# wthanone/kmerLSH

Hardware: AMD Instinct MI355X
Metric: k-mers·iterations/sec (LSH+cluster loop), 10M k-mers × 64 samples (higher is better)
Workload: dtype f32

## Files before the change

kmerlsh_amd/csrc/klsh_engine.cpp:

```cpp
#include <hip/hip_runtime.h>
#include <stdint.h>
#include <stdio.h>
#include <stdlib.h>
#include <stddef.h>
#include <string.h>

#include <algorithm>
#include <array>
#include <atomic>
#include <cstring>
#include <chrono>
#include <cmath>
#include <deque>
#include <functional>
#include <numeric>
#include <string>
#include <thread>
#include <vector>

#include "klsh.h"
#include "klsh_comm.h"
#include "klsh_internal.h"

extern "C" {
// ... 1668 lines not shown
  KLSH_HIP(hipSetDevice(ctx->device));
  std::string err;
  klsh::Comm* c = klsh::make_rccl_comm(rank, world, id, ctx->device, &err);
  if (!c) return fail(KLSH_E_HIP, err);
  c->timeout_s = ctx->comm_timeout_s;
  ctx->release_shard();
  delete ctx->comm;
  ctx->comm = c;
  return 0;
}

int klsh_comm_init_local(klsh_ctx** ctxs, int world) {
  if (!ctxs || world < 1 || world > klsh::kMaxRanks) return fail(KLSH_E_ARG, "bad argument");
  for (int r = 0; r < world; ++r)
    if (!ctxs[r]) return fail(KLSH_E_ARG, "null context");
  std::vector<klsh::Comm*> cs(world);
  klsh::make_local_comms(world, cs.data());
  for (int r = 0; r < world; ++r) {
    ctxs[r]->release_shard();
    delete ctxs[r]->comm;
    ctxs[r]->comm = cs[r];
  }
  return 0;
}

int klsh_set_option(klsh_ctx* ctx, const char* name, int64_t value) {
  if (!ctx || !name) return fail(KLSH_E_ARG, "null argument");
  const std::string n(name);
  auto flag = [&](bool* f) {
    *f = value != 0;
    return 0;
  };
  auto grid = [&](uint32_t* g) {
    if (value < 0 || value > (1 << 20)) return fail(KLSH_E_ARG, n + " must be in [0, 2^20]");
    *g = (uint32_t)value;
    return 0;
  };
  if (n == "shard_min_rows") {
    if (value < 0) return fail(KLSH_E_ARG, "shard_min_rows must be >= 0");
    ctx->shard_min_rows = (uint64_t)value;
    return 0;
  }
  if (n == "phase_timing") return flag(&ctx->phase_timing);
  if (n == "kernel_timing") return flag(&ctx->kernel_timing);
  if (n == "tail_batch") return flag(&ctx->tail_batch);
  if (n == "huge_fold") return flag(&ctx->huge_fold_always);
  if (n == "tail_local") return flag(&ctx->tail_local);
  if (n == "hyperplane_async") {
    if (value != 0 && value != 1) return fail(KLSH_E_ARG, "hyperplane_async must be 0 or 1");
    ctx->hyperplane_async = (uint32_t)value;
    return 0;
  }
  if (n == "hyperplane_window") {
    if (value < 0) return fail(KLSH_E_ARG, "hyperplane_window must be >= 0");
    ctx->hyperplane_window = (uint64_t)value;
    return 0;
  }
  if (n == "progress") {
    if (value < 0 || value > INT32_MAX) return fail(KLSH_E_ARG, "progress must be >= 0");
    ctx->progress = (int)value;
    return 0;
  }
  if (n == "stop_after") {
    if (value < 0 || value > INT32_MAX) return fail(KLSH_E_ARG, "stop_after must be in [0, 2^31)");
    ctx->stop_after = (int)value;
    return 0;
  }
  if (n == "projection") {
    if (value != klsh::kProjAuto && value != klsh::kProjPacked)
      return fail(KLSH_E_ARG, "projection must be 0 (default) or 1 (exact packed chains)");
    KLSH_HIP(hipSetDevice(ctx->device));
    ctx->pw.variant = (uint32_t)value;
    return ctx->apply_projection_variant();
  }
  if (n == "wide_gram") {
    if (value != 0 && value != 8 && value != 16 && value != 32 && value != 64)
      return fail(KLSH_E_ARG, "wide_gram must be 0, 8, 16, 32 or 64");
    ctx->mw.wide_gram = (uint32_t)value;
    return 0;
  }
  if (n == "wide_unrolled") {
    if (value != 0 && value != 1) return fail(KLSH_E_ARG, "wide_unrolled must be 0 or 1");
    ctx->pw.wide_rolled = value ? 0u : 1u;
    return 0;
  }
  if (n == "long_runs") {
    if (value != 0 && value != 1 && value != 4) return fail(KLSH_E_ARG, "long_runs must be 0, 1 or 4");
    ctx->mw.long_off = value == 1 ? 0u : value == 0 ? 1u : 4u;
    KLSH_HIP(hipSetDevice(ctx->device));
    return ctx->cap_slots ? ctx->ensure_long(ctx->cap_slots, ctx->d) : 0;
  }
  if (n == "comm_timeout_s") {
    if (value <= 0) return fail(KLSH_E_ARG, "comm_timeout_s must be > 0");
    ctx->comm_timeout_s = (double)value;
    if (ctx->comm) ctx->comm->timeout_s = (double)value;
    return 0;
  }
  if (n == "kmc_chunk_records") {
    if (value < 0) return fail(KLSH_E_ARG, "kmc_chunk_records must be >= 0");
    ctx->kmc.chunk_records = (uint64_t)value;
    return 0;
  }
  if (n == "kmc_ordinal_base") {
    if (value < 0 || value > (1ll << 48)) return fail(KLSH_E_ARG, "kmc_ordinal_base must be in [0, 2^48]");
    ctx->kmc.ordinal_base = (uint64_t)value;
    return 0;
  }
  if (n == "kmc_keep_first") {
    if (!value) std::vector<uint64_t>().swap(ctx->kmc.first);
    return flag(&ctx->kmc.keep_first);
  }
  if (n == "kcount_batch_reads") {
    if (value < 0) return fail(KLSH_E_ARG, "kcount_batch_reads must be >= 0");
    ctx->kcount.batch_reads = (uint64_t)value;
    return 0;
  }
  if (n == "kcount_table_slots") {
    if (value != 0 && (value < 1024 || value > (1ll << 32) || (value & (value - 1))))
      return fail(KLSH_E_ARG, "kcount_table_slots must be 0 or a power of two in [1024, 2^32]");
    ctx->kcount.table_slots = (uint64_t)value;
    return 0;
  }
  if (n == "kcount_db_prefix") {
    if (value < -1 || value > 15) return fail(KLSH_E_ARG, "kcount_db_prefix must be in [-1, 15]");
    ctx->kcount.db_prefix = (int)value;
    return 0;
  }
  if (n == "kcount_db_chunk_records") {
    if (value < 0) return fail(KLSH_E_ARG, "kcount_db_chunk_records must be >= 0");
    ctx->kcount.db_chunk_records = (uint64_t)value;
    return 0;
  }
  if (n == "kcount_keep_listing") {
    if (!value) {
      std::vector<std::vector<uint64_t>>().swap(ctx->kcount.values);
      std::vector<std::vector<uint32_t>>().swap(ctx->kcount.counts);
    }
    return flag(&ctx->kcount.keep_listing);
  }
  if (n == "h16_grid") return grid(&ctx->pw.h16_grid);
  if (n == "h16_segcap") return grid(&ctx->pw.segcap);
  if (n == "wide_grid") return grid(&ctx->pw.wide_grid);
  if (n == "fix_grid") return grid(&ctx->pw.fix_grid);
  if (n == "small_grid") return grid(&ctx->mw.small_grid);
  if (n == "tail_big_groups") return grid(&ctx->mw.tail_nbig);
  if (n == "tail_small_groups") return grid(&ctx->mw.tail_nsmall);
  if (n == "wide_group_grid") return grid(&ctx->mw.wide_group_grid);
  if (n == "small_screen_grid") return grid(&ctx->mw.screen_grid);
  if (n == "grid_cap") {
    if (int e = grid(&ctx->mw.grid_cap)) return e;
    ctx->kmc.grid_cap = ctx->kcount.grid_cap = ctx->mw.grid_cap;
    return 0;
  }
  if (n == "tail_merge_rows") {
    if (value < 0 || value > (1 << 22)) return fail(KLSH_E_ARG, "tail_merge_rows must be in [0, 2^22]");
    ctx->mw.tail_max = (uint32_t)value;
    return 0;
  }
  if (n == "tail_screen") {
    if (value != 0 && value != 1) return fail(KLSH_E_ARG, "tail_screen must be 0 or 1");
    ctx->mw.tail_screen = (uint32_t)value;
    return 0;
  }
  if (n == "tail_screen_grid") return grid(&ctx->mw.tail_screen_grid);
  if (n == "tail_big_screen") {
    if (value != 0 && value != 1) return fail(KLSH_E_ARG, "tail_big_screen must be 0 or 1");
    ctx->mw.tail_big_screen = (uint32_t)value;
    return 0;
  }
  if (n == "hip_events") {
    if (value != 0 && value != 1) return fail(KLSH_E_ARG, "hip_events must be 0 or 1");
    ctx->hip_events = value != 0;
    return 0;
  }
  if (n == "small_screen") {
    if (value != 0 && value != 1) return fail(KLSH_E_ARG, "small_screen must be 0 or 1");
    ctx->mw.small_screen = (uint32_t)value;
    return 0;
  }
  return fail(KLSH_E_ARG, "unknown option " + n);
}

int klsh_get_option(klsh_ctx* ctx, const char* name, int64_t* value) {
  if (!ctx || !name || !value) return fail(KLSH_E_ARG, "null argument");
  const std::string n(name);
  if (n == "shard_min_rows") *value = (int64_t)ctx->shard_min_rows;
  else if (n == "phase_timing") *value = ctx->phase_timing;
  else if (n == "kernel_timing") *value = ctx->kernel_timing;
  else if (n == "tail_batch") *value = ctx->tail_batch;
  else if (n == "huge_fold") *value = ctx->huge_fold_always;
  else if (n == "tail_local") *value = ctx->tail_local;
  else if (n == "hyperplane_window") *value = (int64_t)ctx->hyperplane_window;
  else if (n == "hyperplane_async") *value = ctx->hyperplane_async;
  else if (n == "stop_after") *value = ctx->stop_after;
  else if (n == "progress") *value = ctx->progress;
  else if (n == "projection") *value = ctx->pw.variant;
  else if (n == "comm_timeout_s") *value = (int64_t)ctx->comm_timeout_s;
  else if (n == "kmc_chunk_records") *value = (int64_t)ctx->kmc.chunk_records;
  else if (n == "kmc_ordinal_base") *value = (int64_t)ctx->kmc.ordinal_base;
  else if (n == "kmc_keep_first") *value = ctx->kmc.keep_first;
  else if (n == "kmc_decode_launches") *value = (int64_t)ctx->kmc.decode_launches;
  else if (n == "kmc_high_sort") *value = ctx->kmc.high_sort;
  else if (n == "kcount_batch_reads") *value = (int64_t)ctx->kcount.batch_reads;
  else if (n == "kcount_table_slots") *value = (int64_t)ctx->kcount.table_slots;
  else if (n == "kcount_keep_listing") *value = ctx->kcount.keep_listing;
  else if (n == "kcount_batches") *value = (int64_t)ctx->kcount.batches;
  else if (n == "kcount_rehashes") *value = (int64_t)ctx->kcount.rehashes;
  else if (n == "kcount_peak_slots") *value = (int64_t)ctx->kcount.peak_slots;
  else if (n == "kcount_window") *value = (int64_t)klsh::kKcountWindow;
  else if (n == "kcount_db_prefix") *value = ctx->kcount.db_prefix;
  else if (n == "kcount_db_chunk_records") *value = (int64_t)ctx->kcount.db_chunk_records;
  else if (n == "kcount_db_chunks") *value = (int64_t)ctx->kcount.db_chunks;
  else if (n == "kcount_db_prefix_used") *value = ctx->kcount.db_prefix_used;
  else if (n == "h16_grid") *value = ctx->pw.h16_grid;
  else if (n == "h16_segcap") *value = ctx->pw.segcap;
  else if (n == "wide_grid") *value = ctx->pw.wide_grid;
  else if (n == "fix_grid") *value = ctx->pw.fix_grid;
  else if (n == "small_grid") *value = ctx->mw.small_grid;
  else if (n == "tail_big_groups") *value = ctx->mw.tail_nbig;
  else if (n == "tail_small_groups") *value = ctx->mw.tail_nsmall;
  else if (n == "wide_group_grid") *value = ctx->mw.wide_group_grid;
  else if (n == "small_screen_grid") *value = ctx->mw.screen_grid;
  else if (n == "grid_cap") *value = ctx->mw.grid_cap;
  else if (n == "tail_merge_rows") *value = klsh::tail_merge_max(ctx->mw);
  else if (n == "small_screen") *value = ctx->mw.small_screen;
  else if (n == "hip_events") *value = ctx->hip_events ? 1 : 0;
  else if (n == "tail_screen") *value = ctx->mw.tail_screen;
  else if (n == "tail_screen_grid") *value = ctx->mw.tail_screen_grid;
  else if (n == "tail_big_screen") *value = ctx->mw.tail_big_screen;
  else if (n == "long_runs") *value = ctx->mw.long_off == 1u ? 0 : ctx->mw.long_off == 0u ? 1 : ctx->mw.long_off;
  else if (n == "wide_gram") *value = ctx->mw.wide_gram;
  else if (n == "wide_unrolled") *value = ctx->pw.wide_rolled ? 0 : 1;
  else if (n == "fp16_image") *value = ctx->rows.xh != nullptr;
  else if (n == "last_hash_kernel") *value = ctx->last_hash_kernel;
  else if (n == "last_hash_close_pairs") *value = (int64_t)ctx->last_hash_close;
  else return fail(KLSH_E_ARG, "unknown option " + n);
  return 0;
}

int klsh_comm_info(klsh_ctx* ctx, int* rank, int* world) {
  if (!ctx) return fail(KLSH_E_ARG, "null ctx");
  if (rank) *rank = ctx->rank();
  if (world) *world = ctx->world();
  return 0;
}

int klsh_count(klsh_ctx* ctx, uint64_t* n_rows, uint64_t* n_members) {
  if (!ctx) return fail(KLSH_E_ARG, "null ctx");
  if (!ctx->loaded) return fail(KLSH_E_STATE, "nothing loaded");
  if (n_rows) *n_rows = ctx->n_live;
  if (n_members) {
    KLSH_HIP(hipSetDevice(ctx->device));
    std::vector<uint32_t> ord(ctx->n_live), cnt(ctx->slots);
    if (ctx->n_live)
      KLSH_HIP(hipMemcpy(ord.data(), ctx->order, 4 * ctx->n_live, hipMemcpyDeviceToHost));
    if (ctx->slots)
      KLSH_HIP(hipMemcpy(cnt.data(), ctx->rows.cnt, 4 * ctx->slots, hipMemcpyDeviceToHost));
    uint64_t m = 0;
    for (uint32_t sl : ord) m += cnt[sl];
    *n_members = m;
  }
  return 0;
}

int klsh_result(klsh_ctx* ctx, float* rows, uint64_t* member_offsets, uint64_t* member_ids) {
  if (!ctx) return fail(KLSH_E_ARG, "null ctx");
  if (!ctx->loaded) return fail(KLSH_E_STATE, "nothing loaded");
  KLSH_HIP(hipSetDevice(ctx->device));
  const uint64_t n = ctx->n_live;
  hipStream_t s = ctx->stream;
  if (rows && n) {
    float* tmp = nullptr;
    if (int e = dalloc(&tmp, n * (uint64_t)ctx->d)) return e;
    klsh::launch_gather_rows(ctx->rows, ctx->order, (uint32_t)n, tmp, s);
    hipError_t e1 = hipMemcpyAsync(rows, tmp, sizeof(float) * n * ctx->d, hipMemcpyDeviceToHost, s);
    hipError_t e2 = hipStreamSynchronize(s);
    dfree(tmp);
    if (e1 != hipSuccess || e2 != hipSuccess) return fail(KLSH_E_HIP, "result rows copy");
  }
  if (member_offsets || member_ids) {
    std::vector<uint32_t> ord(n), head(ctx->slots), nxt(ctx->members);
    if (n) KLSH_HIP(hipMemcpy(ord.data(), ctx->order, 4 * n, hipMemcpyDeviceToHost));
    if (ctx->slots)
      KLSH_HIP(hipMemcpy(head.data(), ctx->rows.head, 4 * ctx->slots, hipMemcpyDeviceToHost));
    if (ctx->members)
      KLSH_HIP(hipMemcpy(nxt.data(), ctx->rows.nxt, 4 * ctx->members, hipMemcpyDeviceToHost));
    uint64_t m = 0;
    for (uint64_t i = 0; i < n; ++i) {
      if (member_offsets) member_offsets[i] = m;
      if (ord[i] >= ctx->slots) return fail(KLSH_E_STATE, "corrupt live order");
      for (uint32_t node = head[ord[i]]; node != klsh::kNil; node = nxt[node]) {
        if (node >= ctx->members || m >= ctx->members)
          return fail(KLSH_E_STATE, "corrupt member list");
        if (member_ids) member_ids[m] = ctx->ids[node];
        ++m;
      }
    }
    if (member_offsets) member_offsets[n] = m;
  }
  return 0;
}

int klsh_row_state(klsh_ctx* ctx, float* nrm, uint32_t* cnt, uint16_t* image,
                   uint64_t* pad_nonzero, uint64_t* bad_links) {
  if (!ctx) return fail(KLSH_E_ARG, "null ctx");
  if (!ctx->loaded) return fail(KLSH_E_STATE, "nothing loaded");
  KLSH_HIP(hipSetDevice(ctx->device));
  KLSH_HIP(hipStreamSynchronize(ctx->stream));
  const uint64_t n = ctx->n_live, S = ctx->slots, M = ctx->members;
  const int d = ctx->d, dp = ctx->dp;
  std::vector<uint32_t> ord(n);
  if (n) KLSH_HIP(hipMemcpy(ord.data(), ctx->order, 4 * n, hipMemcpyDeviceToHost));
  for (uint32_t sl : ord)
    if (sl >= S) return fail(KLSH_E_STATE, "corrupt live order");
  if (nrm && n) {
// ... 289 lines not shown
```

kmerlsh_amd/csrc/klsh_internal.h:

```cpp
#pragma once

#include <hip/hip_ext.h>
#include <hip/hip_runtime_api.h>
#include <stdint.h>
#include <stdio.h>

#include <vector>

#include "klsh.h"

namespace klsh {

constexpr uint32_t kInvalid = 0xFFFFFFFFu;
constexpr uint32_t kNil = 0xFFFFFFFFu;
constexpr int kMaxHyperplanes = 32;
constexpr int kScanTile = 4096;
uint64_t sort_ws_words(uint64_t slots);
constexpr uint32_t kScanStatusWord = 64;
constexpr uint64_t kScanSumsWord = kScanStatusWord + 2ull * (1ull << 20);
inline uint64_t scan_ws_words(uint64_t slots) {
  return kScanSumsWord + (256 * slots) / kScanTile + 1024;
}

constexpr int kBigClasses = 4;
// ... 54 lines not shown
  KStampBlock* blk;
  int set;
  int fold;
  int phase = -1;
};
constexpr KTime kNoTime{nullptr, 0, -1, -1};

struct MergeWork {
  uint2* cls[kGroupClasses];
  uint2* act[kGroupClasses];
  uint32_t screened;
  uint2* big[kBigClasses];
  uint2* huge;
  uint2* over;
  uint32_t* tile_sums;
  RunCounters* rc;
  uint32_t* run_ws;
  uint32_t* dlist;
  uint32_t* mark;
  uint32_t stamp;
  uint32_t big896_aux;
  uint32_t huge_cap;
  uint32_t huge_fold;
  uint64_t* long_P;
  uint32_t long_groups;
  uint32_t long_off = 4;
  uint32_t small_grid;
  uint32_t tail_nbig;
  uint32_t tail_nsmall;
  uint32_t wide_group_grid;
  uint32_t screen_grid;
  uint32_t wide_gram = 32;
  uint32_t small_screen = 1;
  uint32_t tail_screen = 1;
  uint32_t tail_big_screen = 1;
  uint32_t big_screen = 0;
  float bs_s_star = 0.0f, bs_m0 = 0.0f, bs_a2 = 0.0f;
  uint32_t tail_screen_grid;
  uint32_t tail_max;
  uint32_t grid_cap = 0;
  hipStream_t aux[3];
  KTime kt;
  hipEvent_t small_ev[2];
  hipEvent_t fork;
  hipEvent_t join[3];
};
constexpr int kMergeStreams = 3;
inline uint32_t cap_grid(uint32_t g, uint32_t cap) { return cap && g > cap ? cap : g; }
constexpr uint32_t kLongRows = 4096;
inline bool long_ok(int d) { return d == 16 || d == 32; }
inline uint32_t tail_merge_max(const MergeWork& w) { return w.tail_max ? w.tail_max : (1u << 22); }

struct Rows {
  float* x;
  float* nrm;
  uint32_t* cnt;
  uint32_t* head;
  uint32_t* tail;
  uint32_t* nxt;
  int d;
  int dp;
  uint16_t* xh = nullptr;
};
inline bool shadow_width_ok(int d) { return d == 16 || d == 32 || d == 64; }

struct Decider {
  float s_star, s_lo, s_hi;
  uint32_t fast;
  float g_lo, g_hi;
};
constexpr float kGramMargin = 1.0e-4f;
Decider make_decider(float thr);

struct ProjectWork {
  uint2* fix;
  uint32_t* ws;
  uint32_t cap;
  uint32_t h16_grid;
  uint32_t wide_grid;
  uint32_t fix_grid;
  uint32_t segcap;
  uint32_t variant;
  uint32_t wide_rolled;
};
constexpr uint32_t kProjAuto = 0, kProjPacked = 1, kProjScreen = 2;
constexpr uint32_t kH16Grid = 2048;

bool project_device_n_ok(int d);
void launch_project_device_n(const Rows& r, const uint32_t* slots, uint32_t* keys, uint32_t n_max,
                             const float* W, const uint32_t* n_dev, hipStream_t s,
                             KTime kt = kNoTime, const uint32_t* woff_dev = nullptr,
                             const ProjectWork* pw = nullptr);

enum ProjKernel : int { kPkNone = -1, kPkPacked = 0, kPkH16 = 1, kPkWide = 2 };
int launch_project(const Rows& r, const uint32_t* slots, uint32_t* keys, uint32_t n,
                   const float* W, int h, uint32_t key_or, hipStream_t s,
                   const ProjectWork* pw = nullptr, KTime kt = kNoTime);

void radix_sort(uint32_t* k0, uint32_t* v0, uint32_t* k1, uint32_t* v1, uint32_t n, int bits,
                uint32_t* ws, uint32_t** out_k, uint32_t** out_v, hipStream_t s,
                KTime kt = kNoTime, const uint32_t* n_dev = nullptr);

void launch_merge(const Rows& r, const uint32_t* key, uint32_t* slots, uint32_t lo, uint32_t hi,
                  float thr, int bucket_thr, const MergeWork& w, Counters* ctr, hipStream_t s,
                  const uint32_t* n_dev = nullptr, bool runs_ready = false);

const uint32_t* radix_sort_top(const uint32_t* k0, const uint32_t* v0, uint32_t* k1, uint32_t* v1,
                               uint32_t n, int bits, uint32_t* ws, hipStream_t s, KTime kt,
                               const uint32_t* n_dev);
void launch_tail_local(const uint32_t* kin, const uint32_t* vin, uint32_t* kout, uint32_t* vout,
                       const uint32_t* dtot, int bits, int bucket_thr, const MergeWork& w,
                       hipStream_t s);
constexpr int kTailTopBits = 9;
constexpr int kTailLowBits = 19 - kTailTopBits > 10 ? 19 - kTailTopBits : 10;
inline bool tail_local_ok(uint32_t n_max, int bits) {
  return n_max <= (1u << 20) && bits > kTailTopBits && bits <= kTailTopBits + kTailLowBits;
}

constexpr int kRunListCount = kGroupClasses + kBigClasses + 2;
void launch_runs(const uint32_t* key, uint32_t lo, uint32_t n, int bucket_thr, const MergeWork& w,
                 hipStream_t s, const uint32_t* n_dev = nullptr);

struct Publish {
  Counters* host;
  uint32_t* seq_host;
  uint32_t seq;
  uint32_t* n_next;
  uint32_t* woff = nullptr;
};

struct LookBack {
  unsigned long long* status;
  mutable uint32_t epoch;
};

void launch_compact(const uint32_t* slots, uint32_t n, uint32_t* out, uint32_t* tile_sums,
                    Counters* ctr, hipStream_t s, const Publish* pub = nullptr,
                    RunCounters* rc = nullptr, KTime kt = kNoTime,
                    const LookBack* lb = nullptr, const uint32_t* n_dev = nullptr);
void launch_stamp_fold(KStampBlock* blk, int set, hipStream_t s);
void launch_publish_words(const uint32_t* a, uint32_t na, const uint32_t* b, uint32_t nb,
                          uint32_t* dst, uint32_t* seq_host, uint32_t seq, hipStream_t s);

void launch_convert(const Rows& r, const uint16_t* counts, uint32_t bs, const float* lut,
                    const float* v_kmers, uint32_t* keep, uint32_t* order, uint32_t* tile_sums,
                    Counters* ctr, hipStream_t s);

void launch_norms(const Rows& r, uint32_t n, hipStream_t s);
void launch_shadow_build(const Rows& r, uint64_t n, hipStream_t s);


void launch_gather_rows(const Rows& r, const uint32_t* order, uint32_t n, float* out,
                        hipStream_t s);

void launch_fp_selftest(const float* a, const float* b, uint32_t n, float* sqrt_out,
                        float* div_out, hipStream_t s);

constexpr int kMaxBinBits = 12;
constexpr int kMaxRanks = 64;

void launch_bin_hist(const uint32_t* keys, uint32_t n, int shift, uint32_t nbins, uint32_t* hist,
                     hipStream_t s, uint32_t grid_cap = 0);
void launch_bin_split(const uint32_t* hist_all, int world, uint32_t nbins, uint64_t total,
                      uint32_t* owner, uint32_t* cntmat, hipStream_t s);
int launch_partition(const uint32_t* keys, const uint32_t* slots, uint32_t n, int shift,
                     const uint32_t* owner, int world, uint32_t* counts, uint32_t* tile_sums,
// ... 115 lines not shown
```

kmerlsh_amd/csrc/klsh_kernels.hip:

```cpp
#include <hip/hip_runtime.h>

#include <stdlib.h>

#include <string>
#include <type_traits>

#include "klsh_device.h"

namespace klsh {

typedef float f32x2 __attribute__((ext_vector_type(2)));


__device__ __forceinline__ void pk_mac_lo(f32x2& acc, f32x2 w, f32x2 x) {
  f32x2 t;
  asm("v_pk_mul_f32 %1, %2, %3 op_sel_hi:[1,0]\n\tv_pk_add_f32 %0, %0, %1"
      : "+v"(acc), "=&v"(t) : "v"(w), "v"(x));
}
__device__ __forceinline__ void pk_mac_hi(f32x2& acc, f32x2 w, f32x2 x) {
  f32x2 t;
  asm("v_pk_mul_f32 %1, %2, %3 op_sel:[0,1] op_sel_hi:[1,1]\n\tv_pk_add_f32 %0, %0, %1"
      : "+v"(acc), "=&v"(t) : "v"(w), "v"(x));
}

// ... 144 lines not shown
  const int d4 = d & ~3;
  for (int k = 0; k < d4; k += 4) {
    f32x2 x01[RPL], x23[RPL];
#pragma unroll
    for (int r = 0; r < RPL; ++r) {
      const float4 v = *reinterpret_cast<const float4*>(x[r] + k);
      x01[r] = (f32x2){v.x, v.y};
      x23[r] = (f32x2){v.z, v.w};
    }
    column(swq + (size_t)k * nq, x01, false);
    column(swq + (size_t)(k + 1) * nq, x01, true);
    column(swq + (size_t)(k + 2) * nq, x23, false);
    column(swq + (size_t)(k + 3) * nq, x23, true);
  }
  for (int k = d4; k < d; ++k) {
    f32x2 xk[RPL];
#pragma unroll
    for (int r = 0; r < RPL; ++r) xk[r] = (f32x2){x[r][k], x[r][k]};
    column(swq + (size_t)k * nq, xk, false);
  }
#pragma unroll
  for (int r = 0; r < RPL; ++r) {
    uint32_t key = 0;
#pragma unroll
    for (int q = 0; q < QMAX; ++q)
      if (q < nq)
        key = key * 16u + (a[r][q][0].x >= 0.0f ? 8u : 0u) + (a[r][q][0].y >= 0.0f ? 4u : 0u) +
              (a[r][q][1].x >= 0.0f ? 2u : 0u) + (a[r][q][1].y >= 0.0f ? 1u : 0u);
    const uint32_t pr = p0 + 256u * r;
    if (pr < n) keys[pr] = (key >> (uint32_t)(4 * nq - h)) | key_or;
  }
  kt_end(kt, KC_PROJECT);
}

__global__ __launch_bounds__(256) void k_project_generic(const float* __restrict__ X, int d,
                                                         int dp, const uint32_t* __restrict__ slots,
                                                         uint32_t* __restrict__ keys, uint32_t n,
                                                         const float* __restrict__ W, int h,
                                                         uint32_t key_or, KTime kt) {
  kt_fold(kt);
  kt_begin(kt, KC_PROJECT);
  const uint32_t p = blockIdx.x * 256u + threadIdx.x;
  if (p >= n) return;
  const float* x = X + (size_t)slots[p] * dp;
  float s[kMaxHyperplanes];
#pragma unroll
  for (int j = 0; j < kMaxHyperplanes; ++j) s[j] = 0.0f;
  const int d4 = d & ~3;
  for (int k = 0; k < d4; k += 4) {
    const float4 v = *reinterpret_cast<const float4*>(x + k);
#pragma unroll
    for (int j = 0; j < kMaxHyperplanes; ++j) {
      if (j < h) {
        const float* w = W + (size_t)j * dp + k;
        s[j] = s[j] + w[0] * v.x;
        s[j] = s[j] + w[1] * v.y;
        s[j] = s[j] + w[2] * v.z;
        s[j] = s[j] + w[3] * v.w;
      }
    }
  }
  for (int k = d4; k < d; ++k) {
    const float v = x[k];
#pragma unroll
    for (int j = 0; j < kMaxHyperplanes; ++j)
      if (j < h) s[j] = s[j] + W[(size_t)j * dp + k] * v;
  }
  uint32_t key = 0;
#pragma unroll
  for (int j = 0; j < kMaxHyperplanes; ++j)
    if (j < h) key = key * 2u + (s[j] >= 0.0f ? 1u : 0u);
  keys[p] = key | key_or;
  kt_end(kt, KC_PROJECT);
}

typedef float pf32x16 __attribute__((ext_vector_type(16)));

typedef _Float16 ph16x8 __attribute__((ext_vector_type(8)));

float h16_eps(int d) {
  const float ks = (float)((d + 15) / 16);
  return 1.5f * (0x1p-11f + 0x1p-22f + (17.0f + 2.0f * ks) * 0x1p-23f + (float)(d + 1) * 0x1p-24f);
}
float h16_abs(int d) { return 1.5f * 2.0f * 0x1p-25f * std::sqrt((float)d); }

typedef _Float16 ph16x2 __attribute__((ext_vector_type(2)));

template <int D>
__global__ __launch_bounds__(256) __attribute__((amdgpu_waves_per_eu(4))) void k_project_h16(const uint16_t* __restrict__ XH,
                                                     const float* __restrict__ X, int dp,
                                                     const uint32_t* __restrict__ slots,
                                                     uint32_t* __restrict__ keys, uint32_t n,
                                                     const float* __restrict__ W, int h,
                                                     uint32_t key_or, float eps, float abs_c,
                                                     ProjectWork pw, uint32_t segcap, KTime kt,
                                                     const uint32_t* __restrict__ n_dev,
                                                     const uint32_t* __restrict__ woff_dev) {
  constexpr int KS = D / 16;
  __shared__ ph16x8 sa[2][KS][64];
  __shared__ __attribute__((aligned(16))) float swf[32 * D];
  __shared__ float swn[32];
  __shared__ uint32_t s_cnt;
  __shared__ uint32_t s_close;
  kt_fold(kt);
  kt_begin(kt, KC_PROJECT);
  if (n_dev) {
    n = *n_dev;
    h = n ? 31 - __builtin_clz(n) : 0;
    if (woff_dev) W += (size_t)*woff_dev * dp;
  }
  const uint32_t t = threadIdx.x, lane = t & 63u, hh = lane >> 5;
  const uint32_t wv = t >> 6;
  const uint32_t step = gridDim.x * 256u;
  uint32_t g0 = (blockIdx.x * 4u + wv) * 64u;
  auto load_rows = [&](ph16x8 (&xr)[2 * KS], uint32_t sl) __attribute__((always_inline)) {
    const uint16_t* src = XH + (size_t)sl * dp;
#pragma unroll
    for (int c = 0; c < 2 * KS; ++c) xr[c] = *reinterpret_cast<const ph16x8*>(src + 8 * c);
  };
  constexpr int NWL = 32 * D / 256;
  float wl[NWL];
#pragma unroll
  for (int i = 0; i < NWL; ++i) {
    const int e = (int)t + 256 * i, j = e / D, k = e % D;
    wl[i] = W[(size_t)(j < h ? j : 0) * dp + k];
  }
  const uint32_t sl0 = slots[g0 + lane < n ? g0 + lane : 0u];
  __builtin_amdgcn_sched_barrier(0);
  ph16x8 xr[2 * KS];
  load_rows(xr, sl0);
  __builtin_amdgcn_sched_barrier(0);
#pragma unroll
  for (int i = 0; i < NWL; ++i) {
    const int e = (int)t + 256 * i;
    swf[e] = e / D < h ? wl[i] : 0.0f;
  }
  if (t == 0) s_cnt = s_close = 0u;
  __syncthreads();
  {
    const int j = (int)(t >> 3), p = (int)(t & 7u);
    float a = 0.0f;
#pragma unroll
    for (int k = p; k < D; k += 8) a += swf[j * D + k] * swf[j * D + k];
    a += __shfl_xor(a, 1, 64);
    a += __shfl_xor(a, 2, 64);
    a += __shfl_xor(a, 4, 64);
    if (p == 0) swn[j] = __builtin_amdgcn_sqrtf(a) * 1.001f;
  }
  for (int e = (int)t; e < KS * 64; e += 256) {
    const int sk = e >> 6, L = e & 63, j = L & 31, k0 = 16 * sk + 8 * (L >> 5);
    ph16x8 hi8, lo8;
#pragma unroll
    for (int q = 0; q < 8; ++q) {
      const float w = swf[j * D + k0 + q];
      const _Float16 hi = (_Float16)w;
      hi8[q] = hi;
      lo8[q] = (_Float16)(w - (float)hi);
    }
    sa[0][sk][L] = hi8;
    sa[1][sk][L] = lo8;
  }
  __syncthreads();
  uint4* seg = reinterpret_cast<uint4*>(pw.fix) + (size_t)blockIdx.x * segcap;
  auto group = [&](const ph16x8 (&xr)[2 * KS], uint32_t g0) __attribute__((always_inline)) {
    float ss = 0.0f;
#pragma unroll
    for (int c = 0; c < 2 * KS; ++c)
#pragma unroll
      for (int e = 0; e < 8; e += 2) {
        const ph16x2 v = {xr[c][e], xr[c][e + 1]};
        ss = __builtin_amdgcn_fdot2(v, v, ss, false);
      }
    const float xn = __builtin_amdgcn_sqrtf(ss) * 1.001f;
    pf32x16 accA, accB;
#pragma unroll
    for (int i = 0; i < 16; ++i) accA[i] = accB[i] = 0.0f;
#pragma unroll
    for (int sk = 0; sk < KS; ++sk) {
      uint4 a = *reinterpret_cast<const uint4*>(&xr[2 * sk]);
      uint4 b = *reinterpret_cast<const uint4*>(&xr[2 * sk + 1]);
      auto p0 = __builtin_amdgcn_permlane32_swap(a.x, b.x, false, false);
      auto p1 = __builtin_amdgcn_permlane32_swap(a.y, b.y, false, false);
      auto p2 = __builtin_amdgcn_permlane32_swap(a.z, b.z, false, false);
      auto p3 = __builtin_amdgcn_permlane32_swap(a.w, b.w, false, false);
      a = make_uint4(p0[0], p1[0], p2[0], p3[0]);
      b = make_uint4(p0[1], p1[1], p2[1], p3[1]);
      const ph16x8 fa = *reinterpret_cast<const ph16x8*>(&a);
      const ph16x8 fb = *reinterpret_cast<const ph16x8*>(&b);
      const ph16x8 wh = sa[0][sk][lane], wl = sa[1][sk][lane];
      accA = __builtin_amdgcn_mfma_f32_32x32x16_f16(wh, fa, accA, 0, 0, 0);
      accB = __builtin_amdgcn_mfma_f32_32x32x16_f16(wh, fb, accB, 0, 0, 0);
      accA = __builtin_amdgcn_mfma_f32_32x32x16_f16(wl, fa, accA, 0, 0, 0);
      accB = __builtin_amdgcn_mfma_f32_32x32x16_f16(wl, fb, accB, 0, 0, 0);
    }
    const float xo = __shfl_xor(xn, 32, 64);
    uint32_t bits[2], amb[2];
#pragma unroll
    for (int tb = 0; tb < 2; ++tb) {
      const float xr_n = (tb == 0) == (hh == 0) ? xn : xo;
      const float c1 = eps * xr_n + abs_c, c2 = abs_c * xr_n;
      const bool huge = !(xr_n <= 0x1p100f);
      uint32_t bt = 0u, am = 0u;
#pragma unroll
      for (int i = 0; i < 16; ++i) {
        const int j = (i & 3) + 8 * (i >> 2) + 4 * (int)hh;
        if (j < h) {
          const float sv = tb ? accB[i] : accA[i];
          const float bound = swn[j] * c1 + c2;
          bt |= (sv >= 0.0f ? 1u : 0u) << j;
          am |= ((!(__builtin_fabsf(sv) > bound) || huge) ? 1u : 0u) << j;
        }
      }
      bits[tb] = bt | (uint32_t)__shfl_xor((int)bt, 32, 64);
      amb[tb] = am | (uint32_t)__shfl_xor((int)am, 32, 64);
    }
    const uint32_t row = g0 + lane;
    const uint32_t mb = hh ? bits[1] : bits[0], ma = hh ? amb[1] : amb[0];
    if (row < n) {
      uint32_t key_bits = mb & ~ma;
      bool done = true;
      if (ma) {
        atomicAdd(&s_close, (uint32_t)__popc(ma));
        const uint32_t at = atomicAdd(&s_cnt, 1u);
        if (at < segcap) {
          seg[at] = make_uint4(row, ma, key_bits, 0u);
          done = false;
        } else {
          const float* x = X + (size_t)slots[row] * dp;
          uint32_t a = ma;
          while (a) {
            const int j = __builtin_ctz(a);
            a &= a - 1u;
            float sd = 0.0f;
            for (int k = 0; k < D; ++k) sd = sd + swf[j * D + k] * x[k];
            if (sd >= 0.0f) key_bits |= 1u << j;
          }
        }
      }
      if (done) keys[row] = (h > 0 ? (__builtin_bitreverse32(key_bits) >> (32 - h)) : 0u) | key_or;
    }
  };
  while (g0 < n) {
    const uint32_t sl = slots[g0 + step + lane < n ? g0 + step + lane : 0u];
    group(xr, g0);
    g0 += step;
    if (g0 >= n) break;
    load_rows(xr, sl);
  }
  __syncthreads();
  const uint32_t cnt = min(s_cnt, segcap);
  for (uint32_t e = t; e < cnt; e += 256) {
    const uint4 f = seg[e];
    const float* x = X + (size_t)slots[f.x] * dp;
    float4 u[D / 4];
#pragma unroll
    for (int q = 0; q < D / 4; ++q) u[q] = *reinterpret_cast<const float4*>(x + 4 * q);
    uint32_t key_bits = f.z, a = f.y;
    while (a) {
      const int j = __builtin_ctz(a);
      a &= a - 1u;
      const float* w = swf + j * D;
      float sd = 0.0f;
#pragma unroll
      for (int q = 0; q < D / 4; ++q) {
        const float4 v = *reinterpret_cast<const float4*>(w + 4 * q);
        sd = sd + v.x * u[q].x;
        sd = sd + v.y * u[q].y;
        sd = sd + v.z * u[q].z;
        sd = sd + v.w * u[q].w;
      }
      if (sd >= 0.0f) key_bits |= 1u << j;
    }
    keys[f.x] = (h > 0 ? (__builtin_bitreverse32(key_bits) >> (32 - h)) : 0u) | key_or;
  }
  if (t == 0 && s_close)
    atomicAdd(reinterpret_cast<unsigned long long*>(pw.ws + 32 + 2 * (blockIdx.x & 15u)),
              (unsigned long long)s_close);
  kt_end(kt, KC_PROJECT);
}

typedef _Float16 wh16x8 __attribute__((ext_vector_type(8)));
constexpr int kWideNT = 384;

float wide_eps(int d) {
  const float ks = (float)((d + 15) / 16);
  return 1.5f * (3.0f * 0x1p-22f + (17.0f + 3.0f * ks) * 0x1p-23f + (float)(d + 1) * 0x1p-24f);
}
float wide_abs(int d) { return 3.0f * 0x1p-25f * std::sqrt((float)d); }

__device__ __forceinline__ void hsplit8(float4 u, float4 v, wh16x8& hi, wh16x8& lo, wh16x8& ah) {
  const float x[8] = {u.x, u.y, u.z, u.w, v.x, v.y, v.z, v.w};
#pragma unroll
  for (int j = 0; j < 8; ++j) {
    const _Float16 hb = (_Float16)x[j];
    hi[j] = hb;
    lo[j] = (_Float16)(x[j] - (float)hb);
    ah[j] = __builtin_fabsf16(hb);
  }
}

constexpr int kWidePF = 1;
template <int DT>
__global__ __launch_bounds__(kWideNT, 2) void k_project_mfma_wide(const float* __restrict__ X, int d, int dp,
                                                           const uint32_t* __restrict__ slots,
                                                           uint32_t* __restrict__ keys, uint32_t n,
                                                           const float* __restrict__ W, int h,
                                                           uint32_t key_or, float eps, float abs_c,
                                                           ProjectWork pw, KTime kt) {
  extern __shared__ __attribute__((aligned(16))) unsigned char psm[];
  kt_fold(kt);
  kt_begin(kt, KC_PROJECT);
  const int KS = (d + 15) / 16;
  wh16x8* bfr = reinterpret_cast<wh16x8*>(psm);
  float* swn = reinterpret_cast<float*>(psm + (size_t)KS * 64 * 2 * sizeof(wh16x8));
  const uint32_t t = threadIdx.x, lane = t & 63u, wv = t >> 6, r = lane & 31u, hh = lane >> 5;
  if constexpr (DT > 0) {
    constexpr int KSC = DT / 16, NE = (KSC * 64 + kWideNT - 1) / kWideNT;
    __shared__ float wpart[32][kWideNT / 32];
    const int j = (int)(t & 31u), half = (int)((t >> 5) & 1u), jc = j < h ? j : 0;
    float4 wl[NE][2];
#pragma unroll
    for (int u = 0; u < NE; ++u) {
      const int sk = min((int)wv + (int)(kWideNT / 64) * u, KSC - 1);
      const float* src = W + (size_t)jc * dp + 16 * sk + 8 * half;
      wl[u][0] = *reinterpret_cast<const float4*>(src);
      wl[u][1] = *reinterpret_cast<const float4*>(src + 4);
    }
    float sq = 0.0f;
#pragma unroll
    for (int u = 0; u < NE; ++u) {
      const int sk = (int)wv + (int)(kWideNT / 64) * u;
      if (sk < KSC) {
        float x[8] = {wl[u][0].x, wl[u][0].y, wl[u][0].z, wl[u][0].w,
                      wl[u][1].x, wl[u][1].y, wl[u][1].z, wl[u][1].w};
        wh16x8 hi, lo;
#pragma unroll
// ... 167 lines not shown
            float sd = 0.0f;
            for (int q = 0; q < d; ++q) sd = sd + w[q] * x[q];
            const uint32_t bit = 1u << (h - 1 - j);
            keys[row] = sd >= 0.0f ? (keys[row] | bit) : (keys[row] & ~bit);
          }
          ++k;
        }
      }
    }
  }
}

__global__ __launch_bounds__(256) void k_project_fix(const float* __restrict__ X, int d, int dp,
                                                     const uint32_t* __restrict__ slots,
                                                     uint32_t* __restrict__ keys,
                                                     const float* __restrict__ W, int h,
                                                     ProjectWork pw, KTime kt,
                                                     const uint32_t* __restrict__ n_dev = nullptr,
                                                     const uint32_t* __restrict__ woff_dev = nullptr) {
  extern __shared__ __attribute__((aligned(16))) float fw[];
  __shared__ uint32_t s_last;
  if (n_dev) {
    const uint32_t n = *n_dev;
    h = n ? 31 - __builtin_clz(n) : 0;
    if (woff_dev) W += (size_t)*woff_dev * dp;
  }
  const uint32_t count = min(pw.ws[0], pw.cap);
  if (blockIdx.x * 256u < count) {
    const int nv = h * dp / 4;
    const float4* W4 = reinterpret_cast<const float4*>(W);
    float4* fw4 = reinterpret_cast<float4*>(fw);
    constexpr int U = 16;
    for (int i0 = (int)threadIdx.x; i0 < nv; i0 += 256 * U) {
      float4 v[U];
#pragma unroll
      for (int u = 0; u < U; ++u) v[u] = W4[min(i0 + 256 * u, nv - 1)];
#pragma unroll
      for (int u = 0; u < U; ++u) fw4[min(i0 + 256 * u, nv - 1)] = v[u];
    }
  }
  __syncthreads();
  for (uint32_t e = blockIdx.x * 256u + threadIdx.x; e < count; e += gridDim.x * 256u) {
    const uint2 f = pw.fix[e];
    const float* x = X + (size_t)slots[f.x] * dp;
    const float* w = fw + (size_t)f.y * dp;
    float sd = 0.0f;
    int k = 0;
    for (; k + 64 <= d; k += 64) {
      float4 u[16];
#pragma unroll
      for (int q = 0; q < 16; ++q) u[q] = *reinterpret_cast<const float4*>(x + k + 4 * q);
#pragma unroll
      for (int q = 0; q < 16; ++q) {
        const float4 v = *reinterpret_cast<const float4*>(w + k + 4 * q);
        sd = sd + v.x * u[q].x;
        sd = sd + v.y * u[q].y;
        sd = sd + v.z * u[q].z;
        sd = sd + v.w * u[q].w;
      }
    }
    for (; k < d; ++k) sd = sd + w[k] * x[k];
    const uint32_t bit = 1u << (h - 1 - (int)f.y);
    if (sd >= 0.0f) atomicOr(&keys[f.x], bit);
    else atomicAnd(&keys[f.x], ~bit);
  }
  if (threadIdx.x == 0) s_last = atomicAdd(&pw.ws[1], 1u) == gridDim.x - 1 ? 1u : 0u;
  __syncthreads();
  if (s_last && threadIdx.x == 0) {
    atomicAdd(reinterpret_cast<unsigned long long*>(pw.ws + 4), (unsigned long long)pw.ws[0]);
    atomicExch(&pw.ws[0], 0u);
    atomicExch(&pw.ws[1], 0u);
  }
  kt_end(kt, KC_PROJECT);
}

static void launch_h16(const Rows& r, const uint32_t* slots, uint32_t* keys, uint32_t n,
                       const float* W, int h, uint32_t key_or, hipStream_t s,
                       const ProjectWork& pw, KTime kt, const uint32_t* n_dev,
                       const uint32_t* woff_dev) {
  const uint32_t gmax = pw.h16_grid ? pw.h16_grid : kH16Grid;
  const uint32_t grid = std::min<uint32_t>((n + 255) / 256, gmax);
  uint32_t segcap = (pw.cap / 2) / grid;
  if (pw.segcap) segcap = std::min(segcap, pw.segcap);
  const float eps = h16_eps(r.d), abs_c = h16_abs(r.d);
  auto go = [&](auto screen) {
    screen<<<grid, 256, 0, s>>>(r.xh, r.x, r.dp, slots, keys, n, W, h, key_or, eps, abs_c, pw,
                                segcap, kt, n_dev, woff_dev);
  };
  if (r.d == 64) go(k_project_h16<64>);
  else if (r.d == 32) go(k_project_h16<32>);
  else go(k_project_h16<16>);
}

static bool h16_ok(const Rows& r, const ProjectWork* pw) {
  return pw && pw->variant != kProjPacked && r.xh && (r.d == 16 || r.d == 32 || r.d == 64);
}

bool project_device_n_ok(int d) {
  return d == 8 || d == 16 || d == 32 || d == 64;
}

void launch_project_device_n(const Rows& r, const uint32_t* slots, uint32_t* keys, uint32_t n_max,
                             const float* W, const uint32_t* n_dev, hipStream_t s, KTime kt,
                             const uint32_t* woff_dev, const ProjectWork* pw) {
  if (n_max == 0) return;
  if (h16_ok(r, pw)) {
    const int hmax = 31 - __builtin_clz(n_max);
    launch_h16(r, slots, keys, n_max, W, hmax, 0u, s, *pw, kt, n_dev, woff_dev);
    return;
  }
  const dim3 grid((n_max + 255) / 256), block(256);
  auto go = [&](auto kern) {
    kern<<<grid, block, 0, s>>>(r.x, r.dp, slots, keys, n_max, W, 0, 0u, n_dev, kt, woff_dev);
  };
  switch (r.d) {
    case 8: go(k_project_pk<8, 2, 1>); break;
    case 16: go(k_project_pk<16, 2, 1>); break;
    case 32: go(k_project_pk<32, 2, 1>); break;
    default: go(k_project_pk<64, 2, 1>); break;
  }
}

int launch_project(const Rows& r, const uint32_t* slots, uint32_t* keys, uint32_t n,
                    const float* W, int h, uint32_t key_or, hipStream_t s, const ProjectWork* pw,
                    KTime kt) {
  if (n == 0) return kPkNone;
  const dim3 grid((n + 255) / 256), block(256);
  if (pw && pw->variant != kProjPacked && r.d > 64 && h > 0) {
    const size_t lds = (size_t)((r.d + 15) / 16) * 64 * 2 * 16 + 32 * sizeof(float);
    const size_t flds = sizeof(float) * (size_t)h * r.dp;
    if (lds <= 96 * 1024 && flds <= 128 * 1024) {
      static const bool lds_ok =
          hipFuncSetAttribute(reinterpret_cast<const void*>(&k_project_mfma_wide<0>),
                              hipFuncAttributeMaxDynamicSharedMemorySize, 96 * 1024) == hipSuccess &&
          hipFuncSetAttribute(reinterpret_cast<const void*>(&k_project_mfma_wide<512>),
                              hipFuncAttributeMaxDynamicSharedMemorySize, 96 * 1024) == hipSuccess &&
          hipFuncSetAttribute(reinterpret_cast<const void*>(&k_project_fix),
                              hipFuncAttributeMaxDynamicSharedMemorySize, 128 * 1024) == hipSuccess;
      (void)lds_ok;
      const uint32_t groups = (n + kWideNT / 2 - 1) / (kWideNT / 2);
      const uint32_t wcap = pw->wide_grid ? pw->wide_grid : 512u;
      const dim3 gm(std::min<uint32_t>(groups, wcap));
      KTime k1 = kt;
      k1.fold = -1;
      if (r.d == 512 && !pw->wide_rolled)
        k_project_mfma_wide<512><<<gm, dim3(kWideNT), lds, s>>>(r.x, r.d, r.dp, slots, keys, n, W,
                                                                h, key_or, wide_eps(r.d),
                                                                wide_abs(r.d), *pw, kt);
      else
        k_project_mfma_wide<0><<<gm, dim3(kWideNT), lds, s>>>(r.x, r.d, r.dp, slots, keys, n, W, h,
                                                              key_or, wide_eps(r.d), wide_abs(r.d),
                                                              *pw, kt);
      const uint32_t fcap = pw->fix_grid ? pw->fix_grid : 1024u;
      k_project_fix<<<fcap, block, flds, s>>>(r.x, r.d, r.dp, slots, keys, W, h, *pw, k1);
      return kPkWide;
    }
  }
  if (h16_ok(r, pw) && h > 0) {
    launch_h16(r, slots, keys, n, W, h, key_or, s, *pw, kt, nullptr, nullptr);
    return kPkH16;
  }
  auto go_pk = [&](auto kern) {
    kern<<<grid, block, 0, s>>>(r.x, r.dp, slots, keys, n, W, h, key_or, nullptr, kt, nullptr);
  };
  switch (r.d) {
    case 8: go_pk(k_project_pk<8, 2, 1>); break;
    case 16: go_pk(k_project_pk<16, 2, 1>); break;
// ... 347 lines not shown
```

Measured before the change: 28.28 billion.

## Use tighter |W|·|x| error bound in fp16 projection screen to reduce fixups

The fp16 MFMA hashing screen now builds an extra MFMA accumulator of |W_hi|·|x|. This gives a per-entry rounding bound that replaces the coarser norm-based Cauchy-Schwarz bound, so fewer near-zero projections are flagged ambiguous and sent to the exact fp32 fixup path. Cross-half shuffles use permlane32_swap instead of shfl_xor, and the slot index is stored in the fix segment so the fixup pass does not reload slots. The cost is one extra MFMA per k-step, extra LDS, and reordered accumulation; the new bound is on by default (h16_cs=0) and can be switched back with an option.

```diff
diff --git a/kmerlsh_amd/csrc/klsh_engine.cpp b/kmerlsh_amd/csrc/klsh_engine.cpp
--- a/kmerlsh_amd/csrc/klsh_engine.cpp
+++ b/kmerlsh_amd/csrc/klsh_engine.cpp
@@ -1774,6 +1774,11 @@
   if (n == "wide_unrolled") {
     if (value != 0 && value != 1) return fail(KLSH_E_ARG, "wide_unrolled must be 0 or 1");
     ctx->pw.wide_rolled = value ? 0u : 1u;
+    return 0;
+  }
+  if (n == "h16_bound") {
+    if (value != 0 && value != 1) return fail(KLSH_E_ARG, "h16_bound must be 0 or 1");
+    ctx->pw.h16_cs = value ? 0u : 1u;
     return 0;
   }
   if (n == "long_runs") {
@@ -1923,6 +1928,7 @@
   else if (n == "long_runs") *value = ctx->mw.long_off == 1u ? 0 : ctx->mw.long_off == 0u ? 1 : ctx->mw.long_off;
   else if (n == "wide_gram") *value = ctx->mw.wide_gram;
   else if (n == "wide_unrolled") *value = ctx->pw.wide_rolled ? 0 : 1;
+  else if (n == "h16_bound") *value = ctx->pw.h16_cs ? 0 : 1;
   else if (n == "fp16_image") *value = ctx->rows.xh != nullptr;
   else if (n == "last_hash_kernel") *value = ctx->last_hash_kernel;
   else if (n == "last_hash_close_pairs") *value = (int64_t)ctx->last_hash_close;
diff --git a/kmerlsh_amd/csrc/klsh_internal.h b/kmerlsh_amd/csrc/klsh_internal.h
--- a/kmerlsh_amd/csrc/klsh_internal.h
+++ b/kmerlsh_amd/csrc/klsh_internal.h
@@ -160,6 +160,7 @@
   uint32_t segcap;
   uint32_t variant;
   uint32_t wide_rolled;
+  uint32_t h16_cs;
 };
 constexpr uint32_t kProjAuto = 0, kProjPacked = 1, kProjScreen = 2;
 constexpr uint32_t kH16Grid = 2048;
diff --git a/kmerlsh_amd/csrc/klsh_kernels.hip b/kmerlsh_amd/csrc/klsh_kernels.hip
--- a/kmerlsh_amd/csrc/klsh_kernels.hip
+++ b/kmerlsh_amd/csrc/klsh_kernels.hip
@@ -250,6 +250,7 @@
   const float ks = (float)((d + 15) / 16);
   return 1.5f * (0x1p-11f + 0x1p-22f + (17.0f + 2.0f * ks) * 0x1p-23f + (float)(d + 1) * 0x1p-24f);
 }
+float h16_eps_t(int d) { return h16_eps(d) * (1.0f + 0x1p-9f); }
 float h16_abs(int d) { return 1.5f * 2.0f * 0x1p-25f * std::sqrt((float)d); }
 
 typedef _Float16 ph16x2 __attribute__((ext_vector_type(2)));
@@ -265,7 +266,7 @@
                                                      const uint32_t* __restrict__ n_dev,
                                                      const uint32_t* __restrict__ woff_dev) {
   constexpr int KS = D / 16;
-  __shared__ ph16x8 sa[2][KS][64];
+  __shared__ ph16x8 sa[3][KS][64];
   __shared__ __attribute__((aligned(16))) float swf[32 * D];
   __shared__ float swn[32];
   __shared__ uint32_t s_cnt;
@@ -293,10 +294,10 @@
     const int e = (int)t + 256 * i, j = e / D, k = e % D;
     wl[i] = W[(size_t)(j < h ? j : 0) * dp + k];
   }
-  const uint32_t sl0 = slots[g0 + lane < n ? g0 + lane : 0u];
+  uint32_t sl = slots[g0 + lane < n ? g0 + lane : 0u];
   __builtin_amdgcn_sched_barrier(0);
   ph16x8 xr[2 * KS];
-  load_rows(xr, sl0);
+  load_rows(xr, sl);
   __builtin_amdgcn_sched_barrier(0);
 #pragma unroll
   for (int i = 0; i < NWL; ++i) {
@@ -317,20 +318,29 @@
   }
   for (int e = (int)t; e < KS * 64; e += 256) {
     const int sk = e >> 6, L = e & 63, j = L & 31, k0 = 16 * sk + 8 * (L >> 5);
-    ph16x8 hi8, lo8;
+    ph16x8 hi8, lo8, ab8;
 #pragma unroll
     for (int q = 0; q < 8; ++q) {
       const float w = swf[j * D + k0 + q];
       const _Float16 hi = (_Float16)w;
       hi8[q] = hi;
       lo8[q] = (_Float16)(w - (float)hi);
+      ab8[q] = __builtin_fabsf16(hi);
     }
     sa[0][sk][L] = hi8;
     sa[1][sk][L] = lo8;
+    sa[2][sk][L] = ab8;
   }
   __syncthreads();
   uint4* seg = reinterpret_cast<uint4*>(pw.fix) + (size_t)blockIdx.x * segcap;
-  auto group = [&](const ph16x8 (&xr)[2 * KS], uint32_t g0) __attribute__((always_inline)) {
+  auto xor32 = [&](uint32_t v) __attribute__((always_inline)) {
+    auto p = __builtin_amdgcn_permlane32_swap(v, v, false, false);
+    return hh ? p[0] : p[1];
+  };
+  const bool tbound = pw.h16_cs == 0u;
+  const float eps_t = tbound ? eps : 0.0f, eps_n = tbound ? 0.0f : eps;
+  auto group = [&](ph16x8 (&xr)[2 * KS], uint32_t g0, uint32_t slot) __attribute__((always_inline)) {
+    asm volatile("" ::: "memory");
     float ss = 0.0f;
 #pragma unroll
     for (int c = 0; c < 2 * KS; ++c)
@@ -340,47 +350,62 @@
         ss = __builtin_amdgcn_fdot2(v, v, ss, false);
       }
     const float xn = __builtin_amdgcn_sqrtf(ss) * 1.001f;
-    pf32x16 accA, accB;
-#pragma unroll
-    for (int i = 0; i < 16; ++i) accA[i] = accB[i] = 0.0f;
+    const float xo = __uint_as_float(xor32(__float_as_uint(xn)));
 #pragma unroll
     for (int sk = 0; sk < KS; ++sk) {
-      uint4 a = *reinterpret_cast<const uint4*>(&xr[2 * sk]);
-      uint4 b = *reinterpret_cast<const uint4*>(&xr[2 * sk + 1]);
+      const uint4 a = *reinterpret_cast<const uint4*>(&xr[2 * sk]);
+      const uint4 b = *reinterpret_cast<const uint4*>(&xr[2 * sk + 1]);
       auto p0 = __builtin_amdgcn_permlane32_swap(a.x, b.x, false, false);
       auto p1 = __builtin_amdgcn_permlane32_swap(a.y, b.y, false, false);
       auto p2 = __builtin_amdgcn_permlane32_swap(a.z, b.z, false, false);
       auto p3 = __builtin_amdgcn_permlane32_swap(a.w, b.w, false, false);
-      a = make_uint4(p0[0], p1[0], p2[0], p3[0]);
-      b = make_uint4(p0[1], p1[1], p2[1], p3[1]);
-      const ph16x8 fa = *reinterpret_cast<const ph16x8*>(&a);
-      const ph16x8 fb = *reinterpret_cast<const ph16x8*>(&b);
-      const ph16x8 wh = sa[0][sk][lane], wl = sa[1][sk][lane];
-      accA = __builtin_amdgcn_mfma_f32_32x32x16_f16(wh, fa, accA, 0, 0, 0);
-      accB = __builtin_amdgcn_mfma_f32_32x32x16_f16(wh, fb, accB, 0, 0, 0);
-      accA = __builtin_amdgcn_mfma_f32_32x32x16_f16(wl, fa, accA, 0, 0, 0);
-      accB = __builtin_amdgcn_mfma_f32_32x32x16_f16(wl, fb, accB, 0, 0, 0);
-    }
-    const float xo = __shfl_xor(xn, 32, 64);
+      *reinterpret_cast<uint4*>(&xr[2 * sk]) = make_uint4(p0[0], p1[0], p2[0], p3[0]);
+      *reinterpret_cast<uint4*>(&xr[2 * sk + 1]) = make_uint4(p0[1], p1[1], p2[1], p3[1]);
+    }
     uint32_t bits[2], amb[2];
 #pragma unroll
     for (int tb = 0; tb < 2; ++tb) {
+      pf32x16 accS, accT;
+#pragma unroll
+      for (int i = 0; i < 16; ++i) accS[i] = accT[i] = 0.0f;
+      if (tbound) {
+#pragma unroll
+        for (int sk = 0; sk < KS; ++sk) {
+          uint4 u = *reinterpret_cast<const uint4*>(&xr[2 * sk + tb]);
+          const ph16x8 fx = *reinterpret_cast<const ph16x8*>(&u);
+          u.x &= 0x7fff7fffu;
+          u.y &= 0x7fff7fffu;
+          u.z &= 0x7fff7fffu;
+          u.w &= 0x7fff7fffu;
+          const ph16x8 fabs8 = *reinterpret_cast<const ph16x8*>(&u);
+          accS = __builtin_amdgcn_mfma_f32_32x32x16_f16(sa[0][sk][lane], fx, accS, 0, 0, 0);
+          accT = __builtin_amdgcn_mfma_f32_32x32x16_f16(sa[2][sk][lane], fabs8, accT, 0, 0, 0);
+          accS = __builtin_amdgcn_mfma_f32_32x32x16_f16(sa[1][sk][lane], fx, accS, 0, 0, 0);
+        }
+      } else {
+#pragma unroll
+        for (int sk = 0; sk < KS; ++sk) {
+          const ph16x8 fx = xr[2 * sk + tb];
+          accS = __builtin_amdgcn_mfma_f32_32x32x16_f16(sa[0][sk][lane], fx, accS, 0, 0, 0);
+          accS = __builtin_amdgcn_mfma_f32_32x32x16_f16(sa[1][sk][lane], fx, accS, 0, 0, 0);
+        }
+      }
       const float xr_n = (tb == 0) == (hh == 0) ? xn : xo;
-      const float c1 = eps * xr_n + abs_c, c2 = abs_c * xr_n;
+      const float c1 = eps_n * xr_n + abs_c, c2 = abs_c * xr_n;
       const bool huge = !(xr_n <= 0x1p100f);
       uint32_t bt = 0u, am = 0u;
 #pragma unroll
       for (int i = 0; i < 16; ++i) {
         const int j = (i & 3) + 8 * (i >> 2) + 4 * (int)hh;
         if (j < h) {
-          const float sv = tb ? accB[i] : accA[i];
-          const float bound = swn[j] * c1 + c2;
+          const float sv = accS[i], asv = __builtin_fabsf(sv);
+          const float bound = eps_t * accT[i] + (swn[j] * c1 + c2);
           bt |= (sv >= 0.0f ? 1u : 0u) << j;
-          am |= ((!(__builtin_fabsf(sv) > bound) || huge) ? 1u : 0u) << j;
+          am |= ((!(asv > bound) || !(asv <= 0x1.fffffep127f) || huge) ? 1u : 0u) << j;
         }
       }
-      bits[tb] = bt | (uint32_t)__shfl_xor((int)bt, 32, 64);
-      amb[tb] = am | (uint32_t)__shfl_xor((int)am, 32, 64);
+      bits[tb] = bt | xor32(bt);
+      amb[tb] = am | xor32(am);
     }
     const uint32_t row = g0 + lane;
     const uint32_t mb = hh ? bits[1] : bits[0], ma = hh ? amb[1] : amb[0];
@@ -391,15 +416,17 @@
         atomicAdd(&s_close, (uint32_t)__popc(ma));
         const uint32_t at = atomicAdd(&s_cnt, 1u);
         if (at < segcap) {
-          seg[at] = make_uint4(row, ma, key_bits, 0u);
+          seg[at] = make_uint4(row, ma, key_bits, slot);
           done = false;
         } else {
-          const float* x = X + (size_t)slots[row] * dp;
+          const float* x = X + (size_t)slot * dp;
           uint32_t a = ma;
           while (a) {
             const int j = __builtin_ctz(a);
             a &= a - 1u;
+            asm volatile("" ::: "memory");
             float sd = 0.0f;
+#pragma unroll 4
             for (int k = 0; k < D; ++k) sd = sd + swf[j * D + k] * x[k];
             if (sd >= 0.0f) key_bits |= 1u << j;
           }
@@ -409,17 +436,18 @@
     }
   };
   while (g0 < n) {
-    const uint32_t sl = slots[g0 + step + lane < n ? g0 + step + lane : 0u];
-    group(xr, g0);
+    const uint32_t nx = slots[g0 + step + lane < n ? g0 + step + lane : 0u];
+    group(xr, g0, sl);
     g0 += step;
     if (g0 >= n) break;
-    load_rows(xr, sl);
+    load_rows(xr, nx);
+    sl = nx;
   }
   __syncthreads();
   const uint32_t cnt = min(s_cnt, segcap);
   for (uint32_t e = t; e < cnt; e += 256) {
     const uint4 f = seg[e];
-    const float* x = X + (size_t)slots[f.x] * dp;
+    const float* x = X + (size_t)f.w * dp;
     float4 u[D / 4];
 #pragma unroll
     for (int q = 0; q < D / 4; ++q) u[q] = *reinterpret_cast<const float4*>(x + 4 * q);
@@ -753,7 +781,7 @@
   const uint32_t grid = std::min<uint32_t>((n + 255) / 256, gmax);
   uint32_t segcap = (pw.cap / 2) / grid;
   if (pw.segcap) segcap = std::min(segcap, pw.segcap);
-  const float eps = h16_eps(r.d), abs_c = h16_abs(r.d);
+  const float eps = pw.h16_cs ? h16_eps(r.d) : h16_eps_t(r.d), abs_c = h16_abs(r.d);
   auto go = [&](auto screen) {
     screen<<<grid, 256, 0, s>>>(r.xh, r.x, r.dp, slots, keys, n, W, h, key_or, eps, abs_c, pw,
                                 segcap, kt, n_dev, woff_dev);
```

Measured after the change: 28.65 billion (median of 6 runs). 1.01x the previous value.
